# bastienjacquet/CudaDepthMapIntegration

Measured on AMD Instinct MI355X. Metric: Gvoxel-projections/s, higher is better.
Workload: dtype f64

## Files before the change

cudadepthmapintegration_amd/build.py:

```python
from __future__ import annotations

import os
import re
import shutil
import subprocess
from concurrent.futures import ThreadPoolExecutor

_HERE = os.path.dirname(os.path.abspath(__file__))
ROOT = os.path.dirname(_HERE)
CSRC = os.path.join(_HERE, "csrc")
OBJ_DIR = os.path.join(ROOT, "build", "obj")
LIB_PATH = os.path.join(CSRC, "libdmi_hip.so")

SOURCES = ["fusion_kernels.hip", "fusion_tile.hip", "fusion_classify.hip", "coloration_kernels.hip", "mesh_depth_render.hip", "grid_post.hip", "isosurface.hip", "isosurface_components.hip", "isosurface_smooth.hip", "isosurface_decimate.hip", "isosurface_holes.hip", "isosurface_support.hip", "depth_consistency.hip", "scene_bounds.hip", "dmi_capi.hip", "dmi_capi_views.hip", "dmi_capi_fuse.hip", "dmi_capi_mesh.hip", "dmi_capi_color.hip", "dmi_capi_consistency.hip", "dmi_capi_bounds.hip", "dmi_multi.hip", "host/recon_host.cpp", "host/vti_reader.cpp", "host/vtp_reader.cpp", "host/recon_cli.cpp", "host/color_cli.cpp", "host/dmi_host_capi.cpp"]
HEADERS = ["fusion_kernels.h", "view_records.h", "fusion_launch_rules.h", "fusion_device.h", "dmi_buffer.h", "dmi_context.h", "dmi_color_context.h", "coloration_kernels.h", "mesh_depth_render.h", "depth_consistency.h", "scene_bounds.h", "scene_bounds_rules.h", "rounded_quotient.h", "fusion_tile_acc.inc", "isosurface_table.inc", os.path.join("host", "recon_host.h"),
           os.path.join("host", "vtk_xml_data.h"), os.path.join("host", "vti_reader.h"), os.path.join("host", "vtp_reader.h"),
           os.path.join("host", "recon_cli.h"), os.path.join("host", "color_cli.h"), os.path.join("host", "fan_triangulate.h"),
           os.path.join("..", "..", "include", "dmi.h"), os.path.join("..", "..", "include", "dmi_host.h")]
CLI_MAINS = ["recon_cli_main.cpp", "color_cli_main.cpp"]

COMMON_FLAGS = ["-O3", "-std=c++17", "-fPIC", "-ffp-contract=off", "-fno-fast-math", "-Wall", "-Wno-unused-function",
                "-Wno-inline-asm", "-Wno-pass-failed"]
HIP_FLAGS = ["--offload-arch=gfx950", "-mllvm", "-disable-promote-alloca-to-vector", "-Xoffload-linker", "--discard-all"]
OPTIONAL_LLVM_FLAGS = ["-amdgpu-use-amdgpu-trackers=1"]
# ... 135 lines not shown
        name = m.group(1)
        tpl = re.search(r"fuse_tile_kernelI\w\wLi(\d+)ELi(\d)ELi(\d)ELi(\d)ELi(\d)ELb([01])", name)
        tk, minw = int(tpl.group(1)), int(tpl.group(4))
        base = ACC_BASES.get(minw, 128)
        code = body[: body.find("s_endpgm")]
        in_asm = False
        scc_from_asm = False
        for line in code.splitlines():
            if "#ASMSTART" in line:
                in_asm = True
                continue
            if "#ASMEND" in line:
                in_asm = False
                continue
            op = line.split()[0] if line.split() else ""
            if in_asm:
                if op.startswith("s_and_saveexec"):
                    scc_from_asm = True
            elif op.startswith("s_"):
                if scc_from_asm and re.match(r"s_(cbranch_scc|cselect|cmov|addc|subb)", op):
                    bad.append(f"{name}: {op} reads the SCC an asm statement's s_and_saveexec_b64 wrote: {line.strip()}")
                if not re.match(r"s_(mov|movk|load|buffer_load|waitcnt|nop|branch|cbranch|cselect|cmov|getpc|setpc|swappc|sleep|barrier|endpgm)", op):
                    scc_from_asm = False
            elif line.rstrip().endswith(":") and not line.startswith((" ", "\t")):
                scc_from_asm = False
            if in_asm or not re.match(r"\s+(v_|global_|buffer_|ds_|scratch_|flat_)", line):
                continue
            regs = [int(x) for x in re.findall(r"\bv(\d+)\b", line)]
            for a, b in re.findall(r"\bv\[(\d+):(\d+)\]", line):
                regs += [int(a), int(b)]
            if any(r >= base for r in regs):
                bad.append(f"{name}: compiler instruction touches the accumulator file (base v{base}): {line.strip()}")
        d = re.search(r"\.amdhsa_kernel " + re.escape(name) + r"\b.*?\.amdhsa_next_free_vgpr (\d+)", asm_text, re.S)
        if not d:
            bad.append(f"{name}: no kernel descriptor found")
        elif int(d.group(1)) < base + 2 * tk:
            bad.append(f"{name}: descriptor allocates {d.group(1)} VGPRs, the accumulators need {base + 2 * tk}")
        checked += 1
    if checked == 0:
        bad.append("no fuse_tile_kernel instantiation found in the assembly")
    return checked, bad


def scratch_sizes(asm_text: str) -> dict:
    import re

    out = {}
    for m in re.finditer(r"\.amdhsa_kernel (_ZN3dmi\S*fuse_tile_kernel\S*)\b(.*?)\.end_amdhsa_kernel", asm_text, re.S):
        size = re.search(r"\.amdhsa_private_segment_fixed_size (\d+)", m.group(2))
        out[m.group(1)] = int(size.group(1)) if size else 0
    return out


def wait_state_counts(asm_text: str) -> dict:
    import re

    out = {}
    for m in re.finditer(r"^(_ZN3dmi\S*fuse_tile_kernel\S*):.*?\.end_amdhsa_kernel", asm_text, re.S | re.M):
        out[m.group(1)] = len(re.findall(r"^\s*s_nop\b", m.group(0), re.M))
    return out


def _audit_digest() -> str:
    return source_digest([os.path.join(CSRC, "fusion_tile.hip")] + _headers())


def audit_is_current() -> bool:
    import json

    marker = os.path.join(OBJ_DIR, "acc_audit.json")
    try:
        with open(marker) as fh:
            return json.load(fh).get("digest") == _audit_digest()
    except (OSError, ValueError):
        return False


def run_accumulator_audit(verbose: bool = False) -> int:
    import json
    import tempfile

    hipcc = hipcc_path()
    with tempfile.TemporaryDirectory() as tmp:
        out = os.path.join(tmp, "fusion_tile.s")
        cmd = [hipcc] + COMMON_FLAGS + HIP_FLAGS + ["--cuda-device-only", "-S", os.path.join(CSRC, "fusion_tile.hip"), "-o", out]
        if verbose:
            print(" ".join(cmd), flush=True)
        subprocess.check_call(cmd)
        with open(out) as fh:
            text = fh.read()
    checked, bad = audit_accumulator_registers(text)
    scratch = scratch_sizes(text)
    nops = wait_state_counts(text)
    table = {}
    for name, size in scratch.items():
        m = re.search(r"fuse_tile_kernelI(\w)(\w)Li(\d+)ELi(\d)ELi(\d)ELi(\d)ELi(\d)ELb([01])ELb([01])ELb([01])ELb([01])ELb([01])(?:ELb([01]))?E", name)
        if not m:
            continue
        depth, grid, tk, wx, wy, minw, group, count, rot, genk, stay, win, zf = m.groups()
        key = f"depth={depth} grid={grid} tk={tk} waves={wx}x{wy} count={count} rot={rot} genk={genk} stay={stay} win={win} zf={zf or 0}"
        production = depth == "f" and count == "0" and genk == "0" and wx == "1" and wy == "1"
        limit = None if not production else ((16 if "-DDMI_TUNING" in COMMON_FLAGS else 0) if tk == "16" else 48)
        table[key] = {"scratch_bytes_per_lane": size, "production": production, "limit": limit, "s_nop": nops.get(name)}
        if limit is not None and size > limit:
            bad.append(f"{name}: {size} bytes of scratch memory per lane in a production instantiation (limit {limit})")
    if bad:
        raise RuntimeError("accumulator-register audit of fusion_tile.hip FAILED (a toolchain change broke the hidden "
                           "register file; results would be silently wrong):\n  " + "\n  ".join(bad[:20]))
    version = subprocess.run([hipcc, "--version"], capture_output=True, text=True).stdout.strip().splitlines()
    os.makedirs(OBJ_DIR, exist_ok=True)
    with open(os.path.join(OBJ_DIR, "acc_audit.json"), "w") as fh:
        json.dump({"instantiations": checked, "violations": 0, "hipcc": version[:2], "digest": _audit_digest(),
                   "scratch_bytes_per_lane": {"max": max(scratch.values()) if scratch else None,
                                              "instantiations_with_scratch": sum(1 for v in scratch.values() if v),
                                              "production_max": max([v["scratch_bytes_per_lane"] for v in table.values() if v["production"]] or [0])},
                   "instantiation_table": table}, fh, indent=1)
    if verbose:
        print(f"accumulator audit: {checked} fuse_tile_kernel instantiations clean ({version[0] if version else 'hipcc'})", flush=True)
    return checked


def _record(mode: str) -> None:
    import json
    import time

    try:
        os.makedirs(OBJ_DIR, exist_ok=True)
        with open(os.path.join(OBJ_DIR, "build_record.json"), "w") as fh:
            json.dump({"mode": mode, "library": os.path.relpath(LIB_PATH, ROOT), "digest": source_digest(), "time": time.time(),
                       "flags": COMMON_FLAGS + HIP_FLAGS}, fh)
    except OSError:
        pass


def build(force: bool = False, verbose: bool = False) -> str:
    if not force and not needs_build():
        _record("up_to_date: the library's digest file names the present sources and flags; nothing compiled")
        return LIB_PATH
    hipcc = hipcc_path()
    os.makedirs(OBJ_DIR, exist_ok=True)
    headers = _headers()
    digest = source_digest()
    if not force and os.path.exists(LIB_PATH) and os.path.exists(_digest_path()):
        srcs = [os.path.join(CSRC, s) for s in _sources()]
        if not any(_stale(_obj(s), [p] + headers) for s, p in zip(_sources(), srcs)):
            force = True

    def compile_one(src: str):
        path = os.path.join(CSRC, src)
        obj = _obj(src)
        if not force and not _stale(obj, [path] + headers):
            return
        cmd = [hipcc] + COMMON_FLAGS + (HIP_FLAGS if src.endswith(".hip") else []) + ["-c", path, "-o", obj]
        if verbose:
            print(" ".join(cmd), flush=True)
        subprocess.check_call(cmd)

    def audit_if_needed(_):
# ... 54 lines not shown
```

cudadepthmapintegration_amd/csrc/dmi_capi_fuse.hip:

```cpp
#include "dmi_context.h"

#include <algorithm>
#include <cmath>
#include <cstdlib>
#include <cstring>

using dmi::drain_events;
using dmi::EventPair;
using dmi::fail;
using dmi::flush_zero_fill;
using dmi::FuseArgs;
using dmi::FuseConfig;
using dmi::guarded;
using dmi::MapRec;
using dmi::TileArgs;
using dmi::TileMapRec;

namespace {

int sync_maps(dmi_context *ctx) {
  dmi_context::Views &v = ctx->views;
  const size_t n = v.h_maps.size();
  const size_t cap = std::max<size_t>(64, n * 2);
  bool fresh = false;
// ... 232 lines not shown
int tuning_hooks(dmi_context *ctx, TileArgs *out) {
  TileArgs &t = *out;
  if (std::getenv("DMI_DEBUG_NO_DEPTH_LOADS")) t.depth_bytes = 0;
  if (std::getenv("DMI_DEBUG_WG_TIMES")) {
    const size_t per_round = 8 * (size_t)t.xcd_run_wg;
    const size_t blocks = ((size_t)t.super_x * t.super_y * t.super_z * 32 + 32 + per_round - 1) / per_round * per_round;
    const size_t bytes = (blocks * 3 + 2) * sizeof(unsigned long long);
    const int rc = dmi::ensure_idle_buffer(ctx, ctx->tables.wg_times, bytes, bytes);
    if (rc != DMI_OK) return rc;
    ctx->tables.wg_times_blocks = blocks;
    DMI_HIP(ctx, hipMemsetAsync(ctx->tables.wg_times.ptr, 0, bytes, ctx->stream));
    t.wg_times = ctx->tables.wg_times.as<unsigned long long>();
    t.wg_times_n = (int64_t)blocks;
  }
  if (const char *e = std::getenv("DMI_DEBUG_PAIRS")) {
    if (!std::strcmp(e, "nowin")) t.flags |= dmi::TILE_FLAG_DBG_SKIP_WINDOW_PAIRS;
    if (!std::strcmp(e, "onlywin")) t.flags |= dmi::TILE_FLAG_DBG_ONLY_WINDOW_PAIRS;
    if (!std::strcmp(e, "nowinloads")) t.flags |= dmi::TILE_FLAG_DBG_NO_WINDOW_LOADS;
  }
  if (const char *e = std::getenv("DMI_XCD_RUN_WG")) {
    t.xcd_run_wg = std::max(1, std::atoi(e));
    if (((int64_t)t.super_x * t.super_y * t.super_z * 32 + 8 * (int64_t)t.xcd_run_wg) > (int64_t)0x7fffffff)
      return fail(ctx, DMI_ERR_INVALID_ARGUMENT, "dmi_fuse: DMI_XCD_RUN_WG makes the launch too large");
  }
  return DMI_OK;
}
#endif

int tile_tables(dmi_context *ctx, const FuseArgs &a, FuseConfig *cfg, const dmi::TileShape &sh, const dmi::HoleTraits &traits, TileArgs *out) {
  TileArgs &t = *out;
  int rc = cz_table(ctx, a, &t);
  if (rc == DMI_OK) rc = dmi::ensure_buffer(ctx, ctx->tables.queue_heads, 128 * sizeof(int32_t));
  if (rc != DMI_OK) return rc;
  t.queue_heads = ctx->tables.queue_heads.as<int32_t>();
  if (dmi::fuse_without_classes(cfg->variant, (int64_t)t.wbricks_x * t.wbricks_y * (int64_t)t.bricks_z, a.n_maps))
    cfg->variant |= dmi::VAR_NO_BRICK_CLASSES;
  t.class_pitch = dmi::class_table_pitch((int32_t)ctx->views.h_maps.size());
  const bool zero_free = dmi::zero_free(a.init_from_grid != 0, ctx->volume.grid_free_of_negative_zero, ctx->opt.count_hits != 0, cfg->variant);
  if (cfg->variant & dmi::VAR_NO_BRICK_CLASSES) {
    rc = zero_row(ctx, &t);
  } else {
    bool any_tier1 = false;
    for (int32_t m = a.first_map; m < a.first_map + a.n_maps && !any_tier1; ++m) any_tier1 = std::isfinite(ctx->views.h_win_recs[(size_t)m].e_abs);
    dmi::WindowsQuestion q;
    q.tier1 = DMI_TIER1 != 0;
    q.general_k = cfg->general_k != 0;
    q.count_hits = cfg->count_hits != 0;
    q.variant = cfg->variant;
    q.holes = cfg->holes != 0;
    q.many_borders = traits.many_borders;
    q.any_tier1 = any_tier1;
    q.zero_free = zero_free;
    q.depth_f64 = ctx->views.depth_f64;
    rc = class_table(ctx, sh, dmi::use_windows(q), &t);
    if (rc == DMI_OK && !(cfg->variant & dmi::VAR_SPATIAL_ORDER)) rc = order_tables(ctx, sh, cfg->variant, &t);
  }
  if (zero_free) t.behind_mask = 0x0101010101010101ull;
  return rc;
}

int timed_launch(dmi_context *ctx, const FuseArgs &a, const TileArgs &t, const FuseConfig &cfg) {
  EventPair ev;
  if (!ctx->pool.empty()) {
    ev = ctx->pool.back();
    ctx->pool.pop_back();
  } else {
    DMI_HIP(ctx, hipEventCreate(&ev.start));
    DMI_HIP(ctx, hipEventCreate(&ev.stop));
    DMI_HIP(ctx, hipEventCreate(&ev.mid));
  }
  ev.has_mid = cfg.use_tile != 0 && !(cfg.variant & dmi::VAR_NO_BRICK_CLASSES);
  DMI_HIP(ctx, hipEventRecord(ev.start, ctx->stream));
  const dmi_context::LaunchTables &tb = ctx->tables;
  hipError_t e = cfg.use_tile ? dmi::launch_fuse_tiled(t, ctx->views.maps.as<MapRec>(), cfg, ctx->views.pyramid, tb.order_level.as<uint8_t>(),
                                                         tb.classes.ptr ? tb.classes.as<uint8_t>() + tb.coarse_offset : nullptr,
                                                         ev.has_mid ? ev.mid : nullptr, ctx->stream) : dmi::launch_fuse(a, cfg, ctx->stream);
  if (e != hipSuccess) {
    ctx->pool.push_back(ev);
    (void)hipGetLastError();
    return fail(ctx, DMI_ERR_DEVICE, std::string("fusion kernel launch: ") + hipGetErrorString(e));
  }
  DMI_HIP(ctx, hipEventRecord(ev.stop, ctx->stream));
  ctx->pending.push_back(ev);
  return DMI_OK;
}

int fuse_run(dmi_context *ctx, int32_t first, int32_t count, int32_t z_first, int32_t z_count, bool tiled, int run_k_mode,
             bool general_k) {
  DMI_HIP(ctx, hipSetDevice(ctx->opt.device));
  int rc = sync_maps(ctx);
  if (rc != DMI_OK) return rc;
  const bool whole_grid = z_first == 0 && z_count == ctx->grid.cell_dims[2];
  if (!whole_grid) {
    rc = flush_zero_fill(ctx);
    if (rc != DMI_OK) return rc;
  }
  const FuseArgs a = general_args(ctx, first, count, z_first, z_count);

  const dmi::HoleTraits traits = resident_hole_traits(ctx->views);
  FuseConfig cfg;
  cfg.depth_is_f64 = ctx->views.depth_f64 ? 1 : 0;
  cfg.grid_is_f64 = ctx->opt.grid_dtype == DMI_F64 ? 1 : 0;
  cfg.k_mode = run_k_mode;
  cfg.count_hits = ctx->opt.count_hits ? 1 : 0;
  cfg.use_tile = tiled ? 1 : 0;
  cfg.general_k = tiled && general_k ? 1 : 0;
  cfg.holes = traits.holes ? 1 : 0;
// ... 149 lines not shown
```

cudadepthmapintegration_amd/csrc/fusion_launch_rules.h:

```cpp
#pragma once
#include <stddef.h>
#include <stdint.h>

namespace dmi {

constexpr int64_t kNoClassesMaxBricks = 1024;
constexpr int kNoClassesMaxViews = 48;

enum VariantBits : int {
  VAR_EXACT_DIVISION = 1,
  VAR_GENERAL_K = 2,
  VAR_BLOCK_SHAPE_MASK = 12,
  VAR_FORCE_GENERAL = 16,
  VAR_TILE_SHAPE_MASK = 0xE0,
  VAR_TILE_SHAPE_SHIFT = 5,
  VAR_NO_BRICK_CLASSES = 256,
  VAR_SPATIAL_ORDER = 512,
  VAR_FIXED_TILE_SHAPE = 4096,
  VAR_KEEP_BEHIND_ADDS = 1024,
  VAR_NO_INTERIOR = 2048,
  VAR_XCD_RUNS = 8192,
  VAR_ZMAJOR_SLOTS = 16384,
  VAR_PERSISTENT_ALWAYS = 32768,
  VAR_PERSISTENT_NEVER = 65536,
// ... 5 lines not shown
};

constexpr int kCostOrderMaxSlots = 0;

struct HoleTraits {
  bool scattered = false;
  bool holes = false;
  bool tall_by_holes = false;
  bool many_borders = false;
  bool mostly_empty = false;
};

inline HoleTraits hole_traits(unsigned long long mingled, unsigned long long without, unsigned long long strips, unsigned long long pixels) {
  HoleTraits h;
  h.scattered = without <= 6 * mingled;
  h.holes = h.scattered && mingled * 160 > strips;
  h.tall_by_holes = h.scattered && mingled * 80 > strips;
  h.many_borders = mingled * 25 > strips;
  h.tall_by_holes = h.tall_by_holes || h.many_borders;
  if (!h.holes) h.mostly_empty = without * 4 >= pixels && pixels > 0;
  return h;
}

inline int with_default_tile_shape(int variant, bool tiled, const HoleTraits &h, int32_t nx, int32_t ny, int32_t nz) {
  if (tiled && !(variant & (VAR_TILE_SHAPE_MASK | VAR_FIXED_TILE_SHAPE))) {
    const int64_t bricks16 = (int64_t)((nx + 15) / 16) * ((ny + 15) / 16) * ((nz + 15) / 16);
    if (bricks16 <= 32768 && !(h.tall_by_holes && bricks16 >= 4096) && !(h.mostly_empty && bricks16 >= 13824))
      variant |= 7 << VAR_TILE_SHAPE_SHIFT;
  }
  return variant;
}

inline bool fuse_without_classes(int variant, int64_t wave_bricks, int32_t views) {
  if (variant & VAR_NO_BRICK_CLASSES) return true;
  return !(variant & VAR_BRICK_CLASSES_ALWAYS) && wave_bricks <= kNoClassesMaxBricks && views < kNoClassesMaxViews;
}

inline int32_t class_table_pitch(int32_t resident_views) {
  int32_t pitch = 64;
  while (pitch < resident_views) pitch *= 2;
  return pitch;
}

#if defined(__HIP__)
#define DMI_RULES_HD __host__ __device__
#else
#define DMI_RULES_HD
#endif
constexpr int kWinPairBlockViews = 32;
DMI_RULES_HD inline int64_t win_pair_index(int64_t brick, int32_t view, int64_t n_class_bricks) {
  return (((int64_t)(view >> 5) * n_class_bricks + brick) << 5) + (view & 31);
}

inline bool zero_free(bool init_from_grid, bool grid_free_of_negative_zero, bool count_hits, int variant) {
  return (!init_from_grid || grid_free_of_negative_zero) && !count_hits && !(variant & VAR_KEEP_BEHIND_ADDS);
}

struct WindowsQuestion {
  bool tier1;
  bool general_k;
  bool count_hits;
  int variant;
  bool holes, many_borders;
  bool any_tier1;
  bool zero_free;
  bool depth_f64;
};
inline bool use_windows(const WindowsQuestion &q) {
  return q.tier1 && !q.general_k && !q.count_hits && !(q.variant & (VAR_NO_WINDOWS | VAR_NO_INTERIOR)) &&
         (q.holes || q.many_borders || (q.variant & VAR_WINDOWS_ALWAYS)) && q.any_tier1 && q.zero_free && !q.depth_f64;
}

inline bool cost_order(int waves_per_workgroup, int variant, size_t n_slots) {
  return waves_per_workgroup == 1 && !(variant & VAR_NO_COST_ORDER) && ((variant & VAR_COST_ORDER) || n_slots <= (size_t)kCostOrderMaxSlots);
}

}
```

cudadepthmapintegration_amd/csrc/fusion_tile.hip:

```cpp
#include <stdlib.h>

#include <algorithm>
#include <type_traits>

#include "fusion_kernels.h"
#include "fusion_device.h"

#ifndef DMI_T1_CHAINS
#define DMI_T1_CHAINS 4
#endif
#ifndef DMI_T1_COLUMN_CHAINS
#define DMI_T1_COLUMN_CHAINS 2
#endif
#if !defined(DMI_TUNING) && (defined(DMI_EXP_SKIP_WINDOW_VIEWS) || defined(DMI_EXP_SAME_REC) || defined(DMI_EXP_NO_WINDOW_LOADS) || \
                             defined(DMI_EXP_NO_LANE_MARGIN))
#error "a DMI_EXP_* switch that changes results was defined without DMI_TUNING"
#endif

namespace dmi {

int tile_shape_index(int variant);

namespace {

constexpr int kLX = 8, kLY = 8;
typedef unsigned long long mask_t;


#include "fusion_tile_acc.inc"

__device__ __forceinline__ void or_where(uint32_t &bits, mask_t m, uint32_t bit ) {
  mask_t saved;
  asm("s_and_saveexec_b64 %1, %2\n\tv_or_b32 %0, %3, %0\n\ts_mov_b64 exec, %1" : "+v"(bits), "=&s"(saved) : "s"(m), "s"(bit) : "scc");
}

__device__ __forceinline__ mask_t ballot(bool p) { return __builtin_amdgcn_ballot_w64(p); }

template <typename P>
__device__ __forceinline__ P launder(P p) {
  asm volatile("" : "+s"(p));
  return p;
}

__device__ __forceinline__ int pinned_word(int x) {
  asm volatile("" : "+v"(x));
  return __builtin_amdgcn_readfirstlane(x);
}
template <typename T>
__device__ __forceinline__ const T *pinned_ptr(const T *p) {
  const uintptr_t v = reinterpret_cast<uintptr_t>(p);
  const uint32_t lo = (uint32_t)pinned_word((int)(uint32_t)v), hi = (uint32_t)pinned_word((int)(uint32_t)(v >> 32));
  return reinterpret_cast<const T *>(((uintptr_t)hi << 32) | lo);
}
__device__ __forceinline__ double pinned(double x) {
  return __hiloint2double(pinned_word(__double2hiint(x)), pinned_word(__double2loint(x)));
}

__device__ __forceinline__ int cvt_saturating(double x) {
  int r;
  asm("v_cvt_i32_f64 %0, %1" : "=v"(r) : "v"(x));
  return r;
}

typedef float f32x2 __attribute__((ext_vector_type(2)));
__device__ __forceinline__ f32x2 pk_fma_lo0_vs(f32x2 a, f32x2 b, unsigned long long c_bits) {
  f32x2 d;
  asm("v_pk_fma_f32 %0, %1, %2, %3 op_sel_hi:[0,1,1]" : "=v"(d) : "v"(a), "v"(b), "s"(c_bits));
  return d;
}
__device__ __forceinline__ f32x2 pk_fma_hi0_vv(f32x2 a, f32x2 b, f32x2 c) {
  f32x2 d;
  asm("v_pk_fma_f32 %0, %1, %2, %3 op_sel:[1,0,0] op_sel_hi:[1,1,1]" : "=v"(d) : "v"(a), "v"(b), "v"(c));
  return d;
}
__device__ __forceinline__ f32x2 pk_fma_lo0_sv(f32x2 a, unsigned long long b_bits, f32x2 c) {
  f32x2 d;
  asm("v_pk_fma_f32 %0, %1, %2, %3 op_sel_hi:[0,1,1]" : "=v"(d) : "v"(a), "s"(b_bits), "v"(c));
  return d;
}
__device__ __forceinline__ f32x2 pk_fma_hi0_sv(f32x2 a, unsigned long long b_bits, f32x2 c) {
  f32x2 d;
  asm("v_pk_fma_f32 %0, %1, %2, %3 op_sel:[1,0,0] op_sel_hi:[1,1,1]" : "=v"(d) : "v"(a), "s"(b_bits), "v"(c));
  return d;
}
__device__ __forceinline__ f32x2 pk_fnma_slo(f32x2 a, unsigned long long b_bits, f32x2 c) {
  f32x2 d;
  asm("v_pk_fma_f32 %0, %1, %2, %3 op_sel_hi:[1,0,1] neg_lo:[1,0,0] neg_hi:[1,0,0]" : "=v"(d) : "v"(a), "s"(b_bits), "v"(c));
  return d;
}
__device__ __forceinline__ float max_abs(float a, float b) {
  float d;
  asm("v_max_f32 %0, |%1|, |%2|" : "=v"(d) : "v"(a), "v"(b));
  return d;
}
template <int TK>
__device__ __forceinline__ float t1_lane_margin(float cz0, float dcz, float hb, float e1_const, float b) {
  const float cz_last = __builtin_fmaf((float)(TK - 1), dcz, cz0);
  const float least = __builtin_fmaxf(__builtin_fminf(cz0, cz_last), 0x1p-100f);
  const float p = __builtin_fmaf(hb, __builtin_amdgcn_rcpf(least), 1.0f);
  return p < 0x1p21f ? __builtin_fmaf(b, p, e1_const) : __builtin_inff();
}

struct ordered {
  static __device__ __forceinline__ f32x2 pk_fma_s(unsigned long long a_bits, f32x2 b, f32x2 c) {
    f32x2 d;
    asm volatile("v_pk_fma_f32 %0, %1, %2, %3 op_sel_hi:[0,1,1]" : "=v"(d) : "s"(a_bits), "v"(b), "v"(c));
    return d;
  }
  static __device__ __forceinline__ float rcp(float x) {
    float r;
    asm volatile("v_rcp_f32 %0, %1" : "=v"(r) : "v"(x));
    return r;
  }
  static __device__ __forceinline__ float two_minus(float z, float r) {
    float d;
    asm volatile("v_fma_f32 %0, -%1, %2, 2.0" : "=v"(d) : "v"(z), "v"(r));
    return d;
  }
  static __device__ __forceinline__ float mul(float a, float b) {
    float d;
    asm volatile("v_mul_f32 %0, %1, %2" : "=v"(d) : "v"(a), "v"(b));
    return d;
  }
  static __device__ __forceinline__ f32x2 pk_fma_lo_s(f32x2 a, f32x2 b, unsigned long long c_bits) {
    f32x2 d;
    asm volatile("v_pk_fma_f32 %0, %1, %2, %3 op_sel_hi:[1,0,1]" : "=v"(d) : "v"(a), "v"(b), "s"(c_bits));
    return d;
  }
  static __device__ __forceinline__ f32x2 pk_sub_s(f32x2 a, unsigned long long c_bits) {
    f32x2 d;
    asm volatile("v_pk_add_f32 %0, %1, %2 neg_lo:[0,1] neg_hi:[0,1]" : "=v"(d) : "v"(a), "s"(c_bits));
    return d;
  }
  static __device__ __forceinline__ f32x2 pk_fnma_lo(f32x2 a, f32x2 b, f32x2 c) {
    f32x2 d;
    asm volatile("v_pk_fma_f32 %0, %1, %2, %3 op_sel_hi:[1,0,1] neg_lo:[1,0,0] neg_hi:[1,0,0]" : "=v"(d) : "v"(a), "v"(b), "v"(c));
    return d;
  }
  static __device__ __forceinline__ float max_abs(float a, float b) {
    float d;
    asm volatile("v_max_f32 %0, |%1|, |%2|" : "=v"(d) : "v"(a), "v"(b));
    return d;
  }
};
template <size_t S>
__device__ __forceinline__ unsigned scaled_column_bits(float x) {
  static_assert(S == 4 || S == 8, "f32 or f64 depth tables");
  unsigned r;
  if constexpr (S == 4)
    asm("v_fmaak_f32 %0, 4.0, %1, 0x4b400000" : "=v"(r) : "v"(x));
  else
    asm("v_fmaak_f32 %0, 4.0, %1, 0x4b400000" : "=v"(r) : "v"(x + x));
  return r;
}
__device__ __forceinline__ int cvt_i32_f32(float x) {
  int r;
  asm("v_cvt_i32_f32 %0, %1" : "=v"(r) : "v"(x));
  return r;
}

template <typename T>
__device__ __forceinline__ T cload(const T *p) {
  return *reinterpret_cast<const T __attribute__((address_space(4))) *>(reinterpret_cast<uintptr_t>(p));
}

template <typename DepthT>
struct DepthLoad;
template <>
struct DepthLoad<float> {
  typedef float raw_t;
  static __device__ __forceinline__ raw_t load(__amdgpu_buffer_rsrc_t rsrc, unsigned pixel) {
    return __uint_as_float(__builtin_amdgcn_raw_buffer_load_b32(rsrc, (int)(pixel << 2), 0, 0));
  }
  static __device__ __forceinline__ raw_t load_at(__amdgpu_buffer_rsrc_t rsrc, unsigned byte_offset) {
    return __uint_as_float(__builtin_amdgcn_raw_buffer_load_b32(rsrc, (int)byte_offset, 0, 0));
  }
  static __device__ __forceinline__ void opaque(raw_t &d) { asm("" : "+v"(d)); }
  static __device__ __forceinline__ bool is_sentinel(raw_t d) { return d == -1.0f; }
  static __device__ __forceinline__ raw_t sentinel() { return -1.0f; }
  static __device__ __forceinline__ raw_t minus_inf() { return -__builtin_inff(); }
  static __device__ __forceinline__ double widen(raw_t d) { return (double)d; }
};
template <>
struct DepthLoad<double> {
  typedef double raw_t;
  static __device__ __forceinline__ raw_t load(__amdgpu_buffer_rsrc_t rsrc, unsigned pixel) {
    typedef unsigned int u32x2 __attribute__((ext_vector_type(2)));
    const u32x2 raw = __builtin_amdgcn_raw_buffer_load_b64(rsrc, (int)(pixel << 3), 0, 0);
    return __hiloint2double((int)raw.y, (int)raw.x);
  }
  static __device__ __forceinline__ raw_t load_at(__amdgpu_buffer_rsrc_t rsrc, unsigned byte_offset) {
    typedef unsigned int u32x2 __attribute__((ext_vector_type(2)));
    const u32x2 raw = __builtin_amdgcn_raw_buffer_load_b64(rsrc, (int)byte_offset, 0, 0);
    return __hiloint2double((int)raw.y, (int)raw.x);
  }
  static __device__ __forceinline__ void opaque(raw_t &d) { asm("" : "+v"(d)); }
  static __device__ __forceinline__ bool is_sentinel(raw_t d) { return d == -1.0; }
  static __device__ __forceinline__ raw_t sentinel() { return -1.0; }
  static __device__ __forceinline__ raw_t minus_inf() { return -__builtin_inf(); }
  static __device__ __forceinline__ double widen(raw_t d) { return d; }
};

template <typename DepthT>
__device__ __forceinline__ bool tile_exact(const FuseArgs *__restrict__ fa, int m, __amdgpu_buffer_rsrc_t rsrc, int i,
                                           int j, int k, double &val) {
  double g[12], rt[12], kk[12];
  const MapRec *maps = cload(&fa->maps);
#pragma unroll
  for (int q = 0; q < 12; ++q) {
    g[q] = cload(&fa->g[q]);
    rt[q] = cload(&maps[m].rt[q]);
    kk[q] = cload(&maps[m].k[q]);
  }
  const int W = cload(&fa->W), H = cload(&fa->H);
  const double gx = cload(&fa->ox) + (i + 0.5) * cload(&fa->sx);
  const double gy = cload(&fa->oy) + (j + 0.5) * cload(&fa->sy);
  const double gz = cload(&fa->oz) + ((k + cload(&fa->kz0)) + 0.5) * cload(&fa->sz);
// ... 155 lines not shown
  const bool lane_ok = (i < head0[0]) & (j < head0[1]);

  const kernarg_t kg = kb;
  const double gx = kg->ox + (i + 0.5) * kg->sx;
  const double gy = kg->oy + (j + 0.5) * kg->sy;
  const double gz0 = kg->oz + ((k0 + kg->kz0) + 0.5) * kg->sz;
  double gm[12];
#pragma unroll
  for (int q = 0; q < 12; ++q) gm[q] = kg->g[q];
  const double wx = ROT ? gm[0] * gx + gm[1] * gy : row4(gm + 0, gx, gy, gz0);
  const double wy = ROT ? gm[4] * gx + gm[5] * gy : row4(gm + 4, gx, gy, gz0);
  const double wz0 = ROT ? gm[8] * gx + gm[9] * gy : row4(gm + 8, gx, gy, gz0);


  uint32_t nh[COUNT ? TK : 1];
#ifndef DMI_EXP_INIT_ALWAYS_OLD
  if constexpr (!PERSIST) {
    if (kg->init_from_grid) {
      GridT held[TK];
      const int ic = i < head0[0] ? i : head0[0] - 1, jc = j < head0[1] ? j : head0[1] - 1;
      const GridT *column = static_cast<const GridT *>(kg->grid) + ((int64_t)k0 * kg->ny + jc) * kg->nx + ic;
      const int64_t plane_in = (int64_t)kg->ny * kg->nx;
#pragma unroll
      for (int kk = 0; kk < TK; ++kk) held[kk] = column[(int64_t)(kk < kcount ? kk : kcount - 1) * plane_in];
#pragma unroll
      for (int kk = 0; kk < TK; ++kk) acc_set<BASE, TK>(kk, (double)held[kk]);
    } else {
#pragma unroll
      for (int kk = 0; kk < TK; ++kk) acc_set<BASE, TK>(kk, 0.0);
    }
  } else
#endif
  {
#pragma unroll
    for (int kk = 0; kk < TK; ++kk) {
      double v0 = 0.0;
      if (kg->init_from_grid && lane_ok && kk < kcount)
        v0 = (double)static_cast<const GridT *>(kg->grid)[(((int64_t)(k0 + kk)) * kg->ny + j) * kg->nx + i];
      acc_set<BASE, TK>(kk, v0);
    }
  }
  if (COUNT) {
#pragma unroll
    for (int kk = 0; kk < TK; ++kk) nh[kk] = 0;
  }

  const mask_t m_lane_ok_brick = ballot(lane_ok);

  const unsigned long long *crow = reinterpret_cast<const unsigned long long *>(
      KA(classes) + (((int64_t)bz * KA(wbricks_y) + wby) * KA(wbricks_x) + wbx) * (int64_t)KA(class_pitch));

  int n_uniform = (!COUNT && KA(free_sums) != nullptr) ? 0 : -1;
  unsigned long long cnext = cload(crow + (first_map >> 3));
  [[maybe_unused]] uint32_t pair_a = 0, pair_b = 0;
  for (int wbase = first_map & ~7; wbase < m_end; wbase += 8) {
    if constexpr (WIN) {
      if ((wbase & 24) == 0 || wbase == (first_map & ~7)) {
        const kernarg_t ko = KFRESH();
        if (ko->win_origin) {
          typedef uint32_t u32x2 __attribute__((ext_vector_type(2)));
          const uint64_t row_off = (uint64_t)(reinterpret_cast<intptr_t>(crow) - reinterpret_cast<intptr_t>(ko->classes));
#ifdef DMI_WINPAIR_BRICK_MAJOR
          const u32x2 *row = reinterpret_cast<const u32x2 *>(reinterpret_cast<intptr_t>(ko->win_origin) + 16 * (int64_t)row_off) + 2 * (wbase & ~31);
#else
          const uint64_t brick = row_off >> __builtin_ctz((unsigned)ko->class_pitch);
          const uint64_t block_first = (uint64_t)(uint32_t)ko->n_class_bricks * (uint32_t)(wbase >> 5);
          const u32x2 *row = reinterpret_cast<const u32x2 *>(ko->win_origin + ((block_first + brick) << 5));
#endif
          const u32x2 pr = row[lane];
          pair_a = pr.x;
          pair_b = pr.y;
        }
      }
    }
    const unsigned long long cword = cnext | ((cnext >> 1) & (ZF ? 0x0101010101010101ull : KC(behind_mask)));
    if (wbase + 8 < m_end) cnext = cload(crow + (wbase >> 3) + 1);
    const unsigned long long nonskip = cword ^ 0x0303030303030303ull;
    unsigned long long todo = (nonskip | (nonskip >> 1)) & 0x0101010101010101ull;
    if (wbase < first_map) todo &= ~0ull << ((first_map - wbase) * 8);
    if (wbase + 8 > m_end) todo &= (1ull << ((m_end - wbase) * 8)) - 1;
    unsigned long long fr = COUNT ? 0ull : (todo & cword & ~(cword >> 1));
    unsigned long long other = todo ^ fr;
  for (;;) {
    const unsigned long long below = (other - 1) & ~other;
    const int n_free_now = __builtin_popcountll(fr & below);
    fr &= ~below;
    if (n_uniform >= 0) {
      n_uniform += n_free_now;
    } else {
      for (int n_free = n_free_now; n_free > 0; --n_free) {
#pragma unroll
        for (int q = 0; q < TK; q += 8) acc_add8_all<BASE, TK>(q, free_space);
      }
    }
    if (other == 0) break;
    const int vbit = __builtin_ctzll(other);
    other &= other - 1;
    const int m = wbase + (vbit >> 3);
    if (n_uniform >= 0) {
      const double v = cload(KC(free_sums) + n_uniform);
#pragma unroll
      for (int q = 0; q < TK; ++q) acc_set<BASE, TK>(q, v);
      n_uniform = -1;
    }
    const unsigned cbyte = (unsigned)(cword >> vbit) & 0x3fu;
    const unsigned cls = cbyte & 3u;
    if (cls != BRICK_MIXED) {
      const double v = cls == BRICK_FREE ? free_space : 0.0;
#pragma unroll
      for (int q = 0; q < TK; q += 8) acc_add8_all<BASE, TK>(q, v);
      if (COUNT) {
#pragma unroll
        for (int q = 0; q < TK; ++q) nh[q] += lane_ok ? 1u : 0u;
        const uint32_t hits = (uint32_t)__popcll(m_lane_ok_brick) * (uint32_t)kcount;
        if (hits != 0 && lane == 0) atomicAdd(&KC(map_hits)[m], (unsigned long long)hits);
      }
      continue;
    }
    [[maybe_unused]] const bool has_window = WIN && cbyte == ((unsigned)MIXED_FREE_OR_NODEPTH << 2 | BRICK_MIXED) && kcount == TK;
#ifdef DMI_TUNING
    ++dbg_cols;
    if ((kflags & TILE_FLAG_DBG_SKIP_WINDOW_PAIRS) && has_window) continue;
    if ((kflags & TILE_FLAG_DBG_ONLY_WINDOW_PAIRS) && !has_window) continue;
#endif
    if constexpr (WIN) {
      if (has_window) {
#ifdef DMI_TUNING
        ++dbg_win;
        if (dbg_cols == dbg_win) ++dbg_win_early;
#endif
        const int pl = (m & 31) * 2;
        const uint32_t org = (uint32_t)__builtin_amdgcn_readlane((int)pair_a, pl);
        const unsigned long long A2 = (unsigned long long)(uint32_t)__builtin_amdgcn_readlane((int)pair_b, pl) |
                                      ((unsigned long long)(uint32_t)__builtin_amdgcn_readlane((int)pair_a, pl + 1) << 32);
        const float acz = __int_as_float(__builtin_amdgcn_readlane((int)pair_b, pl + 1));
        const int x0p = (int)(org & 0xffffu), y0p = (int)(org >> 16);
        const kernarg_t kw = KFRESH();
        typedef uint32_t u32x16 __attribute__((ext_vector_type(16)));
        const WinRec *const wrec = kw->win_recs + m;
        const u32x16 R = *reinterpret_cast<const u32x16 __attribute__((address_space(4))) *>(reinterpret_cast<uintptr_t>(wrec));
#ifndef DMI_NO_WINREC_PREFETCH
        int next_rec;
        asm volatile("s_load_dword %0, %1, 0x40" : "=&s"(next_rec) : "s"(wrec), "s"(R[15]));
#endif
        const __amdgpu_buffer_rsrc_t brsrc = __builtin_amdgcn_make_buffer_rsrc(
            reinterpret_cast<uint32_t *>((uintptr_t)R[0] | ((uintptr_t)R[1] << 32)), (short)0, kw->vb_bytes, 0x00020000);
        const unsigned lin = ((unsigned)lane << 2) + ((unsigned)y0p << 2);
        const unsigned off = __umul24(lin >> 7, (unsigned)kw->vb_rowskip) + lin + (((unsigned)x0p >> 5) << 7);
#ifdef DMI_TUNING
        uint32_t w_lo, w_hi;
        if (kflags & TILE_FLAG_DBG_NO_WINDOW_LOADS) {
          w_lo = off * 0x9e3779b9u, w_hi = ~w_lo;
        } else {
          w_lo = (uint32_t)__builtin_amdgcn_raw_buffer_load_b32(brsrc, (int)off, 0, 0);
          w_hi = (uint32_t)__builtin_amdgcn_raw_buffer_load_b32(brsrc, (int)(off + 128u), 0, 0);
        }
#else
        const uint32_t w_lo = (uint32_t)__builtin_amdgcn_raw_buffer_load_b32(brsrc, (int)off, 0, 0);
        const uint32_t w_hi = (uint32_t)__builtin_amdgcn_raw_buffer_load_b32(brsrc, (int)(off + 128u), 0, 0);
#endif
        const int x0c = x0p - kw->win_cx, y0c = y0p - kw->win_cy;
        f32x2 O, LJ;
        O.x = (float)(x0c + kWinAnchorX);
        O.y = (float)(y0c + kWinAnchorY);
        LJ.x = (float)(lane & 7);
        LJ.y = (float)(lane >> 3);
        auto pair_of = [&](int q) __attribute__((always_inline)) { return (unsigned long long)R[q] | ((unsigned long long)R[q + 1] << 32); };
        auto vec_of = [&](int q) __attribute__((always_inline)) {
          f32x2 v;
          v.x = __uint_as_float(R[q]);
          v.y = __uint_as_float(R[q + 1]);
          asm volatile("" : "+v"(v));
          return v;
        };
        const f32x2 Bwi = pk_fnma_slo(O, pair_of(8), vec_of(2));
        const f32x2 Bwj = pk_fnma_slo(O, pair_of(10), vec_of(4));
        const f32x2 DH = pk_fnma_slo(O, pair_of(12), vec_of(6));
        const f32x2 H0 = pk_fma_hi0_vv(LJ, Bwj, pk_fma_lo0_vs(LJ, Bwi, A2));
        f32x2 CA;
        CA.x = acz;
        CA.y = __builtin_fmaf(acz, __uint_as_float(R[15]), -__uint_as_float(R[14]));
        const f32x2 C0 = pk_fma_hi0_sv(LJ, pair_of(10), pk_fma_lo0_sv(LJ, pair_of(8), CA));
        const f32x2 DC = vec_of(12);
        unsigned long long M2 = (0x4B400000ull + (unsigned)kWinAnchorX) | ((0x4B400000ull + (unsigned)kWinAnchorY) << 32);
        asm volatile("" : "+s"(M2));
        float magic_v = 0x1.8p23f + (float)(4 * kWinAnchorY);
        asm volatile("" : "+v"(magic_v));
        auto first_voxel = [&](double &hxf, double &hyf, double &czf64) __attribute__((always_inline)) {
          const kernarg_t kf = KFRESH();
          const TileMapRec *rf = kf->tile_maps + m;
          double wxf = wx, wyf = wy, wzf = wz0;
          if constexpr (ROT) {
            const czvec4 b = cload(reinterpret_cast<const czvec4 *>(kf->cz_table + (int64_t)k0 * 4));
            wxf = (wx + b[0]) + kf->g[3], wyf = (wy + b[1]) + kf->g[7], wzf = (wz0 + b[2]) + kf->g[11];
            czf64 = ((cload(&rf->rz0) * wxf + cload(&rf->rz1) * wyf) + cload(&kf->maps[m].rt[10]) * wzf) + cload(&rf->rz3);
          } else {
            czf64 = ((cload(&rf->rz0) * wx + cload(&rf->rz1) * wy) + cload(kf->cz_table + (int64_t)m * kf->kpad + k0)) + cload(&rf->rz3);
          }
          hxf = __builtin_fma(cload(&rf->cpx), wxf, __builtin_fma(cload(&rf->cpy), wyf, __builtin_fma(cload(&rf->cpz), wzf, cload(&rf->cp0))));
          hyf = __builtin_fma(cload(&rf->cqx), wxf, __builtin_fma(cload(&rf->cqy), wyf, __builtin_fma(cload(&rf->cqz), wzf, cload(&rf->cq0))));
        };
        uint32_t undecided = 0, und_kk = 0;
        uint32_t window = 0;
        constexpr int WG = 4;
#ifdef DMI_T1_RCP_EVERY_VOXEL
        constexpr bool kNewton = false;
#else
        constexpr bool kNewton = true;
#endif
        [[maybe_unused]] f32x2 r_below;
        uint32_t pw[WG], pc[WG];
        auto consume = [&](int g0) __attribute__((always_inline)) {
          __builtin_amdgcn_s_waitcnt(0xc07f);
          if ((und_kk >> g0) & ((1u << WG) - 1u)) {
  #pragma unroll
            for (int q = 0; q < WG; ++q) pw[q] &= ((undecided >> (g0 + q)) & 1u) - 1u;
          }
  #pragma unroll
          for (int q = 0; q < WG; ++q) {
            int mbit;
            asm("v_bfe_i32 %0, %1, %2, 1" : "=v"(mbit) : "v"(pw[q]), "v"(pc[q]));
            acc_fma_vs<BASE, TK>(g0 + q, __hiloint2double(mbit & 0x3ff00000, 0), free_space);
          }
        };
  #pragma unroll
        for (int g0 = 0; g0 < TK; g0 += WG) {
          uint32_t wg[WG], cg[WG];
          mask_t m_und[WG];
          constexpr int IL = DMI_T1_CHAINS;
          if constexpr (kNewton) {
            static_assert(WG == 4, "the link order below is written for groups of four");
// ... 592 lines not shown
          grid[gid] = sum;
        if (COUNT) ke->voxel_hits[gid] += nh[kk];
      }
      gid += plane;
    }
  }
  if constexpr (!PERSIST) break;
  }
}
#undef DMI_NEXT_BRICK
#undef KA
#undef KC
#undef KFRESH

__global__ __launch_bounds__(256) void launch_tables_kernel(const TileArgs a, const MapRec *__restrict__ maps) {
  fill_launch_tables(a, maps, (int64_t)blockIdx.x * blockDim.x + threadIdx.x, (int64_t)gridDim.x * blockDim.x);
}

constexpr int kPersistentMinViews = 96;

template <typename Kernel>
unsigned resident_workgroups(Kernel kernel, int threads) {
  int device = 0, per_cu = 0;
  hipDeviceProp_t prop;
  if (hipGetDevice(&device) != hipSuccess || hipGetDeviceProperties(&prop, device) != hipSuccess ||
      hipOccupancyMaxActiveBlocksPerMultiprocessor(&per_cu, kernel, threads, 0) != hipSuccess || per_cu <= 0 ||
      prop.multiProcessorCount <= 0) {
    (void)hipGetLastError();
    return 8192u;
  }
  return (unsigned)(per_cu * prop.multiProcessorCount + 7) / 8u * 8u;
}

template <typename DepthT, typename GridT, int TK, int WX, int WY, int MINW, int GROUP, bool ROT = false, bool GENK = false, bool WIN = false>
hipError_t launch_shape(const TileArgs &a, const FuseConfig &cfg, hipStream_t s) {
  static_assert(TK <= kMaxColumnHeight, "dmi_multi_z_slab aligns slabs to kMaxColumnHeight");
  constexpr bool one_wave = WX * WY == 1;
  constexpr bool rare = std::is_same<DepthT, double>::value || GENK;
  static_assert(!WIN || (one_wave && !rare), "window launches are production launches");
  const int per_round = 8 * a.xcd_run_wg;
  unsigned blocks = (unsigned)((a.super_x * a.super_y * a.super_z * 32 + 32 + per_round - 1) / per_round * per_round);
  const dim3 block(64 * WX * WY);
  const bool zf = a.behind_mask != 0 && !cfg.count_hits;
  if (WIN && !zf) return hipErrorInvalidValue;
  bool stay = true;
  if constexpr (one_wave && !rare) {
    const int64_t voxels = (int64_t)a.super_x * a.super_y * a.super_z * 32 * 64 * TK;
    stay = (cfg.variant & VAR_PERSISTENT_ALWAYS) ? true
           : (cfg.variant & VAR_PERSISTENT_NEVER) ? false
           : (cfg.variant & VAR_NO_BRICK_CLASSES) ? true
           : cfg.holes ? (a.n_maps >= 48 && voxels >= (int64_t(1) << 25))
                       : (a.n_maps >= kPersistentMinViews && voxels >= (int64_t(1) << 27));
  }
  auto launch = [&](auto kernel, bool persistent) {
    unsigned n = blocks;
    if (persistent && one_wave) {
      static const unsigned resident = resident_workgroups(kernel, 64);
      n = std::min(n, resident);
    }
    hipLaunchKernelGGL(kernel, dim3(n), block, 0, s, a);
    return hipGetLastError();
  };
  if constexpr (!WIN) {
    if (cfg.count_hits) return launch(fuse_tile_kernel<DepthT, GridT, TK, WX, WY, MINW, GROUP, true, ROT, GENK>, true);
  }
  if constexpr (one_wave && !rare) {
    if (zf) {
      if (!stay) return launch(fuse_tile_kernel<DepthT, GridT, TK, WX, WY, MINW, GROUP, false, ROT, GENK, false, WIN, true>, false);
      return launch(fuse_tile_kernel<DepthT, GridT, TK, WX, WY, MINW, GROUP, false, ROT, GENK, true, WIN, true>, true);
    }
  }
  if constexpr (!WIN) return launch(fuse_tile_kernel<DepthT, GridT, TK, WX, WY, MINW, GROUP, false, ROT, GENK>, true);
  return hipErrorInvalidValue;
}

int effective_shape(int variant, bool depth_is_f64, bool rotated, bool general_k = false) {
  int shape = tile_shape_index(variant);
#ifndef DMI_TUNING
  shape = (shape == 1 || shape == 3 || shape == 4 || shape == 7) ? 7 : 0;
#endif
  if (general_k || depth_is_f64) return 0;
  return (rotated && shape != 7) ? 0 : shape;
}

template <typename DepthT, typename GridT, int TK, int MINW, bool ROT>
hipError_t launch_win(const TileArgs &a, const FuseConfig &cfg, hipStream_t s) {
  if constexpr (DMI_TIER1 != 0 && std::is_same<DepthT, float>::value)
    return launch_shape<DepthT, GridT, TK, 1, 1, MINW, 8, ROT, false, true>(a, cfg, s);
  else
    return hipErrorInvalidValue;
}

template <typename DepthT, typename GridT>
hipError_t launch_types(const TileArgs &a, const FuseConfig &cfg, hipStream_t s) {
  constexpr bool f32_depth = std::is_same<DepthT, float>::value;
  const int shape = effective_shape(cfg.variant, !f32_depth, a.rotated != 0, cfg.general_k != 0);
  const bool win = DMI_TIER1 != 0 && std::is_same<DepthT, float>::value && a.win_origin != nullptr && !cfg.count_hits && !cfg.general_k &&
                   a.behind_mask != 0;
#ifdef DMI_FAST_BUILD
  if (win) {
    if (shape == 7) return launch_win<DepthT, GridT, 8, 6, false>(a, cfg, s);
    return launch_win<DepthT, GridT, 16, 5, false>(a, cfg, s);
  }
  if constexpr (f32_depth) {
    if (shape == 7) return launch_shape<DepthT, GridT, 8, 1, 1, 6, 8>(a, cfg, s);
  }
  return launch_shape<DepthT, GridT, 16, 1, 1, 5, 8>(a, cfg, s);
#else
  if (cfg.general_k) {
    if (a.rotated) return launch_shape<DepthT, GridT, 16, 1, 1, 5, 8, true, true>(a, cfg, s);
    return launch_shape<DepthT, GridT, 16, 1, 1, 5, 8, false, true>(a, cfg, s);
  }
  if (a.rotated) {
    if (win) {
      if (shape == 7) return launch_win<DepthT, GridT, 8, 6, true>(a, cfg, s);
      return launch_win<DepthT, GridT, 16, 5, true>(a, cfg, s);
    }
    if constexpr (f32_depth) {
      if (shape == 7) return launch_shape<DepthT, GridT, 8, 1, 1, 6, 8, true>(a, cfg, s);
    }
    return launch_shape<DepthT, GridT, 16, 1, 1, 5, 8, true>(a, cfg, s);
  }
#ifdef DMI_TUNING
  if constexpr (std::is_same<DepthT, float>::value) {
    switch (shape) {
// ... 90 lines not shown
```

Before: 3106.

## Stage window pair entries in LDS via buffer_load-to-LDS instead of lane registers

By default (without DMI_WINPAIR_LANE_HELD), the per-view window pair entries (origin, A2, acz) are loaded into a 4 KB LDS area. Each 256-view group is filled with buffer_load_dwordx4 ... lds, and entries are read from LDS per map instead of via readlane from lane-held registers. This is meant to cut refills and register pressure, but adds LDS use per workgroup, a vmcnt wait before each read and a different FMA operand form. The host disables windows when the brick count is too large for the buffer addressing, and the build audit now checks that LDS use fits the CU's occupancy.

Measured after the change: 3156, median of 6. 1.02x the previous value.

```diff
diff --git a/cudadepthmapintegration_amd/build.py b/cudadepthmapintegration_amd/build.py
--- a/cudadepthmapintegration_amd/build.py
+++ b/cudadepthmapintegration_amd/build.py
@@ -211,6 +211,14 @@
     return out
 
 
+def lds_sizes(asm_text: str) -> dict:
+    out = {}
+    for m in re.finditer(r"\.amdhsa_kernel (_ZN3dmi\S*fuse_tile_kernel\S*)\b(.*?)\.end_amdhsa_kernel", asm_text, re.S):
+        size = re.search(r"\.amdhsa_group_segment_fixed_size (\d+)", m.group(2))
+        out[m.group(1)] = int(size.group(1)) if size else 0
+    return out
+
+
 def wait_state_counts(asm_text: str) -> dict:
     import re
 
@@ -251,6 +259,7 @@
     checked, bad = audit_accumulator_registers(text)
     scratch = scratch_sizes(text)
     nops = wait_state_counts(text)
+    lds = lds_sizes(text)
     table = {}
     for name, size in scratch.items():
         m = re.search(r"fuse_tile_kernelI(\w)(\w)Li(\d+)ELi(\d)ELi(\d)ELi(\d)ELi(\d)ELb([01])ELb([01])ELb([01])ELb([01])ELb([01])(?:ELb([01]))?E", name)
@@ -260,9 +269,13 @@
         key = f"depth={depth} grid={grid} tk={tk} waves={wx}x{wy} count={count} rot={rot} genk={genk} stay={stay} win={win} zf={zf or 0}"
         production = depth == "f" and count == "0" and genk == "0" and wx == "1" and wy == "1"
         limit = None if not production else ((16 if "-DDMI_TUNING" in COMMON_FLAGS else 0) if tk == "16" else 48)
-        table[key] = {"scratch_bytes_per_lane": size, "production": production, "limit": limit, "s_nop": nops.get(name)}
+        table[key] = {"scratch_bytes_per_lane": size, "production": production, "limit": limit, "s_nop": nops.get(name),
+                      "lds_bytes_per_workgroup": lds.get(name, 0)}
         if limit is not None and size > limit:
             bad.append(f"{name}: {size} bytes of scratch memory per lane in a production instantiation (limit {limit})")
+        waves_per_cu = 4 * (4 if tk == "16" else 5)
+        if production and lds.get(name, 0) * waves_per_cu > 160 * 1024:
+            bad.append(f"{name}: {lds[name]} bytes of LDS per one-wave workgroup: {waves_per_cu} of them do not fit a CU's 160 KB")
     if bad:
         raise RuntimeError("accumulator-register audit of fusion_tile.hip FAILED (a toolchain change broke the hidden "
                            "register file; results would be silently wrong):\n  " + "\n  ".join(bad[:20]))
diff --git a/cudadepthmapintegration_amd/csrc/dmi_capi_fuse.hip b/cudadepthmapintegration_amd/csrc/dmi_capi_fuse.hip
--- a/cudadepthmapintegration_amd/csrc/dmi_capi_fuse.hip
+++ b/cudadepthmapintegration_amd/csrc/dmi_capi_fuse.hip
@@ -308,7 +308,8 @@
     q.any_tier1 = any_tier1;
     q.zero_free = zero_free;
     q.depth_f64 = ctx->views.depth_f64;
-    rc = class_table(ctx, sh, dmi::use_windows(q), &t);
+    const bool windows = dmi::use_windows(q) && dmi::win_pair_pieces_addressable((int64_t)t.wbricks_x * t.wbricks_y * t.bricks_z);
+    rc = class_table(ctx, sh, windows, &t);
     if (rc == DMI_OK && !(cfg->variant & dmi::VAR_SPATIAL_ORDER)) rc = order_tables(ctx, sh, cfg->variant, &t);
   }
   if (zero_free) t.behind_mask = 0x0101010101010101ull;
diff --git a/cudadepthmapintegration_amd/csrc/fusion_launch_rules.h b/cudadepthmapintegration_amd/csrc/fusion_launch_rules.h
--- a/cudadepthmapintegration_amd/csrc/fusion_launch_rules.h
+++ b/cudadepthmapintegration_amd/csrc/fusion_launch_rules.h
@@ -81,6 +81,21 @@
   return (((int64_t)(view >> 5) * n_class_bricks + brick) << 5) + (view & 31);
 }
 
+inline bool win_pair_pieces_addressable(int64_t n_class_bricks) { return n_class_bricks < (int64_t(1) << 22); }
+struct WinPairFill {
+  uint64_t first;
+  uint32_t range;
+};
+DMI_RULES_HD inline uint64_t win_pair_piece_stride(uint64_t n_class_bricks) { return n_class_bricks << 9; }
+DMI_RULES_HD inline WinPairFill win_pair_fill(uint64_t brick, uint32_t block, uint64_t n_class_bricks, uint32_t class_pitch) {
+  const uint64_t table_bytes = (n_class_bricks * class_pitch) << 4;
+  WinPairFill f;
+  f.first = (n_class_bricks * block + brick) << 9;
+  const uint64_t rest = table_bytes > f.first ? table_bytes - f.first : 0;
+  f.range = rest > 0xffffffffull ? 0xffffffffu : (uint32_t)rest;
+  return f;
+}
+
 inline bool zero_free(bool init_from_grid, bool grid_free_of_negative_zero, bool count_hits, int variant) {
   return (!init_from_grid || grid_free_of_negative_zero) && !count_hits && !(variant & VAR_KEEP_BEHIND_ADDS);
 }
diff --git a/cudadepthmapintegration_amd/csrc/fusion_tile.hip b/cudadepthmapintegration_amd/csrc/fusion_tile.hip
--- a/cudadepthmapintegration_amd/csrc/fusion_tile.hip
+++ b/cudadepthmapintegration_amd/csrc/fusion_tile.hip
@@ -66,6 +66,11 @@
 __device__ __forceinline__ f32x2 pk_fma_lo0_vs(f32x2 a, f32x2 b, unsigned long long c_bits) {
   f32x2 d;
   asm("v_pk_fma_f32 %0, %1, %2, %3 op_sel_hi:[0,1,1]" : "=v"(d) : "v"(a), "v"(b), "s"(c_bits));
+  return d;
+}
+__device__ __forceinline__ f32x2 pk_fma_lo0_vv(f32x2 a, f32x2 b, f32x2 c) {
+  f32x2 d;
+  asm("v_pk_fma_f32 %0, %1, %2, %3 op_sel_hi:[0,1,1]" : "=v"(d) : "v"(a), "v"(b), "v"(c));
   return d;
 }
 __device__ __forceinline__ f32x2 pk_fma_hi0_vv(f32x2 a, f32x2 b, f32x2 c) {
@@ -163,6 +168,31 @@
 __device__ __forceinline__ T cload(const T *p) {
   return *reinterpret_cast<const T __attribute__((address_space(4))) *>(reinterpret_cast<uintptr_t>(p));
 }
+
+#if defined(DMI_WINPAIR_BRICK_MAJOR) && !defined(DMI_WINPAIR_LANE_HELD)
+#error "-DDMI_WINPAIR_BRICK_MAJOR (the [brick][view] pair table) is built with the lane-held entries only: add -DDMI_WINPAIR_LANE_HELD"
+#endif
+constexpr int kPairGroupViews = 256;
+typedef uint32_t u32x4 __attribute__((ext_vector_type(4)));
+typedef const u32x4 __attribute__((address_space(3))) *pair_area_t;
+__device__ __forceinline__ pair_area_t pair_area() {
+  __shared__ u32x4 area[kPairGroupViews];
+  return (pair_area_t)area;
+}
+__device__ __forceinline__ void pair_area_load(u32x4 rsrc , unsigned voff, unsigned lds_dst ) {
+  unsigned keep;
+  asm volatile(
+      "s_waitcnt lgkmcnt(0)\n\t"
+      "s_mov_b32 %0, m0\n\t"
+      "s_mov_b32 m0, %2\n\t"
+      "s_nop 4\n\t"
+      "buffer_load_dwordx4 %1, %3, 0 offen lds\n\t"
+      "s_mov_b32 m0, %0"
+      : "=&s"(keep)
+      : "v"(voff), "s"(lds_dst), "s"(rsrc)
+      : "memory");
+}
+__device__ __forceinline__ void pair_area_wait() { asm volatile("s_waitcnt vmcnt(0)" ::: "memory"); }
 
 template <typename DepthT>
 struct DepthLoad;
@@ -424,8 +454,37 @@
 
   int n_uniform = (!COUNT && KA(free_sums) != nullptr) ? 0 : -1;
   unsigned long long cnext = cload(crow + (first_map >> 3));
+#ifdef DMI_WINPAIR_LANE_HELD
   [[maybe_unused]] uint32_t pair_a = 0, pair_b = 0;
+#endif
   for (int wbase = first_map & ~7; wbase < m_end; wbase += 8) {
+#ifndef DMI_WINPAIR_LANE_HELD
+    if constexpr (WIN) {
+      if ((wbase & (kPairGroupViews - 8)) == 0 || wbase == (first_map & ~7)) {
+        const kernarg_t ko = KFRESH();
+        if (ko->win_origin) {
+          const uint64_t row_off = (uint64_t)(reinterpret_cast<intptr_t>(crow) - reinterpret_cast<intptr_t>(ko->classes));
+          const uint64_t brick = row_off >> __builtin_ctz((unsigned)ko->class_pitch);
+          const uint64_t n_bricks = (uint64_t)(uint32_t)ko->n_class_bricks;
+          const uint64_t table = reinterpret_cast<uint64_t>(ko->win_origin);
+          const unsigned voff = ((unsigned)(lane & 31) << 4) + ((lane & 32) ? (unsigned)win_pair_piece_stride(n_bricks) : 0u);
+          const unsigned area0 = (unsigned)reinterpret_cast<uintptr_t>(pair_area());
+          const unsigned block0 = (unsigned)(wbase >> 8) << 3;
+#pragma unroll
+          for (int q = 0; q < kPairGroupViews / 64; ++q) {
+            const WinPairFill f = win_pair_fill(brick, block0 + 2u * (unsigned)q, n_bricks, (uint32_t)ko->class_pitch);
+            const uint64_t base = table + f.first;
+            u32x4 rsrc;
+            rsrc.x = (uint32_t)base;
+            rsrc.y = (uint32_t)(base >> 32) & 0xffffu;
+            rsrc.z = f.range;
+            rsrc.w = 0x00020000u;
+            pair_area_load(rsrc, voff, area0 + 1024u * (unsigned)q);
+          }
+        }
+      }
+    }
+#else
     if constexpr (WIN) {
       if ((wbase & 24) == 0 || wbase == (first_map & ~7)) {
         const kernarg_t ko = KFRESH();
@@ -445,6 +504,7 @@
         }
       }
     }
+#endif
     const unsigned long long cword = cnext | ((cnext >> 1) & (ZF ? 0x0101010101010101ull : KC(behind_mask)));
     if (wbase + 8 < m_end) cnext = cload(crow + (wbase >> 3) + 1);
     const unsigned long long nonskip = cword ^ 0x0303030303030303ull;
@@ -501,11 +561,21 @@
         ++dbg_win;
         if (dbg_cols == dbg_win) ++dbg_win_early;
 #endif
+#ifdef DMI_WINPAIR_LANE_HELD
         const int pl = (m & 31) * 2;
         const uint32_t org = (uint32_t)__builtin_amdgcn_readlane((int)pair_a, pl);
         const unsigned long long A2 = (unsigned long long)(uint32_t)__builtin_amdgcn_readlane((int)pair_b, pl) |
                                       ((unsigned long long)(uint32_t)__builtin_amdgcn_readlane((int)pair_a, pl + 1) << 32);
         const float acz = __int_as_float(__builtin_amdgcn_readlane((int)pair_b, pl + 1));
+#else
+        pair_area_wait();
+        const u32x4 entry = pair_area()[m & (kPairGroupViews - 1)];
+        const uint32_t org = (uint32_t)__builtin_amdgcn_readfirstlane((int)entry.x);
+        f32x2 A2;
+        A2.x = __uint_as_float(entry.y);
+        A2.y = __uint_as_float(entry.z);
+        const float acz = __uint_as_float(entry.w);
+#endif
         const int x0p = (int)(org & 0xffffu), y0p = (int)(org >> 16);
         const kernarg_t kw = KFRESH();
         typedef uint32_t u32x16 __attribute__((ext_vector_type(16)));
@@ -548,7 +618,11 @@
         const f32x2 Bwi = pk_fnma_slo(O, pair_of(8), vec_of(2));
         const f32x2 Bwj = pk_fnma_slo(O, pair_of(10), vec_of(4));
         const f32x2 DH = pk_fnma_slo(O, pair_of(12), vec_of(6));
+#ifdef DMI_WINPAIR_LANE_HELD
         const f32x2 H0 = pk_fma_hi0_vv(LJ, Bwj, pk_fma_lo0_vs(LJ, Bwi, A2));
+#else
+        const f32x2 H0 = pk_fma_hi0_vv(LJ, Bwj, pk_fma_lo0_vv(LJ, Bwi, A2));
+#endif
         f32x2 CA;
         CA.x = acz;
         CA.y = __builtin_fmaf(acz, __uint_as_float(R[15]), -__uint_as_float(R[14]));
@@ -1247,25 +1321,30 @@
            : cfg.holes ? (a.n_maps >= 48 && voxels >= (int64_t(1) << 25))
                        : (a.n_maps >= kPersistentMinViews && voxels >= (int64_t(1) << 27));
   }
-  auto launch = [&](auto kernel, bool persistent) {
+  auto launch = [&](auto kernel, bool persistent, auto which) {
     unsigned n = blocks;
     if (persistent && one_wave) {
       static const unsigned resident = resident_workgroups(kernel, 64);
       n = std::min(n, resident);
     }
+    (void)which;
     hipLaunchKernelGGL(kernel, dim3(n), block, 0, s, a);
     return hipGetLastError();
   };
+  typedef std::integral_constant<int, 0> counted_t;
+  typedef std::integral_constant<int, 1> per_brick_t;
+  typedef std::integral_constant<int, 2> persistent_t;
+  typedef std::integral_constant<int, 3> general_t;
   if constexpr (!WIN) {
-    if (cfg.count_hits) return launch(fuse_tile_kernel<DepthT, GridT, TK, WX, WY, MINW, GROUP, true, ROT, GENK>, true);
+    if (cfg.count_hits) return launch(fuse_tile_kernel<DepthT, GridT, TK, WX, WY, MINW, GROUP, true, ROT, GENK>, true, counted_t{});
   }
   if constexpr (one_wave && !rare) {
     if (zf) {
-      if (!stay) return launch(fuse_tile_kernel<DepthT, GridT, TK, WX, WY, MINW, GROUP, false, ROT, GENK, false, WIN, true>, false);
-      return launch(fuse_tile_kernel<DepthT, GridT, TK, WX, WY, MINW, GROUP, false, ROT, GENK, true, WIN, true>, true);
-    }
-  }
-  if constexpr (!WIN) return launch(fuse_tile_kernel<DepthT, GridT, TK, WX, WY, MINW, GROUP, false, ROT, GENK>, true);
+      if (!stay) return launch(fuse_tile_kernel<DepthT, GridT, TK, WX, WY, MINW, GROUP, false, ROT, GENK, false, WIN, true>, false, per_brick_t{});
+      return launch(fuse_tile_kernel<DepthT, GridT, TK, WX, WY, MINW, GROUP, false, ROT, GENK, true, WIN, true>, true, persistent_t{});
+    }
+  }
+  if constexpr (!WIN) return launch(fuse_tile_kernel<DepthT, GridT, TK, WX, WY, MINW, GROUP, false, ROT, GENK>, true, general_t{});
   return hipErrorInvalidValue;
 }
 
```
